# letitiabanana/PnP-OVSS

Measured on AMD Instinct MI355X. Metric: images/sec (336^2, drop_iter=4, blur+CRF), higher is better.
Workload: dtype bf16x3

## Files before the change

### pnp-ovss_amd/csrc/gemm_x3.hip

```cpp
#include <mutex>
#include <type_traits>

#include "common.h"
#include "gemm.h"
#include "gemm_wide.h"

namespace pnp {

typedef __attribute__((ext_vector_type(4))) uint32_t frag16;

__device__ __forceinline__ void x3_half(f32x4& c0, f32x4& c1, const frag16& ah, const frag16& al, const frag16& bh0, const frag16& bh1,
                                        const frag16& bl0, const frag16& bl1) {
    asm volatile(
        "v_mfma_f32_16x16x32_bf16 %0, %6, %2, %0\n\t"
        "v_mfma_f32_16x16x32_bf16 %1, %7, %2, %1\n\t"
        "v_mfma_f32_16x16x32_bf16 %0, %4, %3, %0\n\t"
        "v_mfma_f32_16x16x32_bf16 %1, %5, %3, %1\n\t"
        "v_mfma_f32_16x16x32_bf16 %0, %4, %2, %0\n\t"
        "v_mfma_f32_16x16x32_bf16 %1, %5, %2, %1"
        : "+v"(c0), "+v"(c1)
        : "v"(ah), "v"(al), "v"(bh0), "v"(bh1), "v"(bl0), "v"(bl1));
}

typedef __attribute__((ext_vector_type(4))) uint32_t u32x4;
typedef __attribute__((address_space(1))) uint32_t gu32;
constexpr int kSkAux = 16;

template <int EPI, bool SK>
__global__ __launch_bounds__(512) void gemm_nt_x3_kernel(const GemmArgs g) {
    constexpr int BM = 256, BN = 256, SLOT = 65536, ARR = 16384;
    constexpr int JM = 8, IN = 4;
    constexpr int NDMA = 8;
    constexpr int kDrain = (EPI == WIDE_GELU_SPLIT || EPI == WIDE_SPLIT) ? 32 : 24;
    constexpr int SROW = kWideStageRow;
    extern __shared__ __attribute__((aligned(16))) char smem[];

    const int tid = threadIdx.x;
    const int lane = tid & 63, wave = __builtin_amdgcn_readfirstlane(tid >> 6);
    const int r = lane & 15, q = lane >> 4;
    const int wm = wave >> 2, wn = wave & 3;
    const int nbm = (g.M + BM - 1) / BM, nbn = g.N / BN;
    const int ntiles = nbm * nbn;
    const int nk = g.K / 32;
    const char* Ab = reinterpret_cast<const char*>(g.A);
    const char* Bb = reinterpret_cast<const char*>(g.B);
    const char* Alo = reinterpret_cast<const char*>(g.A_lo);
    const char* Blo = reinterpret_cast<const char*>(g.B_lo);

    uint32_t soff[4];
    auto set_tile = [&](int tile, int& m0, int& n0, int lane) {
        int bm, bn;
        tile_coords<4>(tile, nbm, nbn, bm, bn);
        m0 = bm * BM;
        n0 = bn * BN;
        const uint32_t lda_b = (uint32_t)g.lda * 2, ldb_b = (uint32_t)g.ldb * 2;
        const int c = (lane & 3) ^ ((-(lane >> 4)) & 3);
#pragma unroll
        for (int i = 0; i < 2; i++) {
            const int row = (wave * 2 + i) * 16 + (lane >> 2);
            int gr = m0 + row;
            gr = gr < g.M ? gr : g.M - 1;
            soff[i] = (uint32_t)gr * lda_b + c * 16;
            gr = n0 + row;
            gr = gr < g.Nvalid ? gr : g.Nvalid - 1;
            soff[2 + i] = (uint32_t)gr * ldb_b + c * 16;
        }
    };
    auto issue_one = [&](int kt, int i, uint32_t on) {
        const int op = i >> 2, rg = (i >> 1) & 1, lo = i & 1;
        const char* base = op ? (lo ? Blo : Bb) : (lo ? Alo : Ab);
        const int d = (kt & 1) * SLOT + op * (2 * ARR) + lo * ARR + (wave * 2 + rg) * 1024;
        const uint32_t lds = (uint32_t)(uintptr_t)(__attribute__((address_space(3))) char*)(smem + d);
        uint32_t voff;
        uint64_t saved;
        asm volatile(
            "s_mov_b64 %1, exec\n\t"
            "s_cmp_lg_u32 %6, 0\n\t"
            "s_cselect_b64 exec, exec, 0\n\t"
            "v_add_u32 %0, %3, %2\n\t"
            "s_mov_b32 m0, %5\n\t"
            "s_nop 0\n\t"
            "global_load_lds_dwordx4 %0, %4\n\t"
            "s_mov_b64 exec, %1"
            : "=&v"(voff), "=&s"(saved)
            : "v"(soff[op * 2 + rg]), "s"((uint32_t)kt * 64), "s"(base), "s"(lds), "s"(on)
            : "memory", "scc");
    };
    auto stamp_sk = [&](int slot) {
        if (g.stamps && tid == 0) {
            g.stamps[((size_t)gridDim.x + blockIdx.x) * 8 + slot] = __builtin_readcyclecounter();
            g.stamps[((size_t)gridDim.x + blockIdx.x) * 8 + 4 + slot] = wall_clock64();
        }
    };
    auto stamp = [&](int slot) {
        if (g.stamps && tid == 0) {
            g.stamps[(size_t)blockIdx.x * 8 + slot] = __builtin_readcyclecounter();
            g.stamps[(size_t)blockIdx.x * 8 + 4 + slot] = wall_clock64();
        }
    };

    const int fo = r * 64 + ((q ^ ((-(r >> 2)) & 3)) << 4);
    int fa_off[2], fb_off[2];
    fa_off[0] = wm * (128 * 64) + fo;
    fb_off[0] = 2 * ARR + wn * (64 * 64) + fo;
    fa_off[1] = fa_off[0] + SLOT;
    fb_off[1] = fb_off[0] + SLOT;
    asm volatile("" : "+v"(fa_off[1]), "+v"(fb_off[1]));
    float* const stg = reinterpret_cast<float*>(smem + SLOT) + wave * (32 * SROW);

    const int bid = blockIdx.x;
    enum { kWhole = 0, kProduce = 1, kOwn = 2 };
    auto get_work = [&](int wi, int& t, int& k0, int& k1, int& kind) {
        const int grid = gridDim.x;
        const int full = SK ? g.sk_full : ntiles;
        t = bid + wi * grid;
        if (t < full) {
            k0 = 0;
            k1 = nk;
            kind = kWhole;
            return true;
        }
        if constexpr (SK) {
            const int j = wi - g.sk_full / grid;
            const int nk2 = nk >> 1;
            const int T = (ntiles - full) * nk2;
            const int u0 = bid * g.sk_upw;
            const int u1 = u0 + g.sk_upw < T ? u0 + g.sk_upw : T;
            if (u0 >= u1 || j > 1) return false;
            const int ta = u0 / nk2, bnd = (ta + 1) * nk2;
            const bool owns = u1 >= bnd, two = u1 > bnd;
            if (j == 0 && (two || !owns)) {
                t = full + ta + (two ? 1 : 0);
                k0 = two ? 0 : 2 * (u0 - ta * nk2);
                k1 = 2 * (u1 - (two ? bnd : ta * nk2));
                kind = kProduce;
                return true;
            }
            if (owns && (j == 0 || two)) {
                t = full + ta;
                k0 = 2 * (u0 - ta * nk2);
                k1 = nk;
                kind = k0 ? kOwn : kWhole;
                return true;
            }
        }
        return false;
    };
    int wi = 0, tile, k0, k1, kind;
    if (!get_work(0, tile, k0, k1, kind)) return;
    int m0, n0;
    bool drain32 = false;
    stamp(0);
    set_tile(tile, m0, n0, lane);
#pragma unroll
    for (int i = 0; i < NDMA; i++) issue_one(k0, i, 1u);

    for (;;) {
        f32x4 acc[JM][IN];
#pragma unroll
        for (int j = 0; j < JM; j++)
#pragma unroll
            for (int i = 0; i < IN; i++) acc[j][i] = f32x4{0.f, 0.f, 0.f, 0.f};

        frag16 ah[4], al[4], bh[2][IN], bl[2][IN];
        auto rd_a = [&](int slot, int s, int jm) {
            const char* p = smem + fa_off[s] + jm * 1024;
            ah[slot] = *reinterpret_cast<const frag16*>(p);
            al[slot] = *reinterpret_cast<const frag16*>(p + ARR);
        };
        auto rd_b = [&](int set, int s, int in) {
            const char* p = smem + fb_off[s] + in * 1024;
            bh[set][in] = *reinterpret_cast<const frag16*>(p);
            bl[set][in] = *reinterpret_cast<const frag16*>(p + ARR);
        };

        if (drain32) PNP_WAIT_VM(kDrain);
        else PNP_WAIT_VM(0);
        __builtin_amdgcn_s_barrier();
#pragma unroll
        for (int i = 0; i < NDMA; i++) issue_one(k0 + 1, i, 1u);
        rd_a(0, 0, 0);
        rd_a(1, 0, 1);
        rd_a(2, 0, 2);
#pragma unroll
        for (int i = 0; i < IN; i++) rd_b(0, 0, i);

        auto slab = [&](int kt, auto par) {
            constexpr int S = decltype(par)::value;
            const uint32_t head = __builtin_amdgcn_readfirstlane((kt >= k0 + 1 && kt + 1 < k1) ? 1 : 0);
            const uint32_t tail = __builtin_amdgcn_readfirstlane((kt + 2 < k1) ? 1 : 0);
#pragma unroll
            for (int j = 0; j < JM; j++) {
                x3_half(acc[j][0], acc[j][1], ah[j & 3], al[j & 3], bh[S][0], bh[S][1], bl[S][0], bl[S][1]);
                if (j + 3 < JM) {
                    rd_a((j + 3) & 3, S, j + 3);
                    if (j < 2) issue_one(kt + 1, 4 + 2 * j, head);
                } else {
                    if (j == JM - 3) {
                        __builtin_amdgcn_s_waitcnt(0x0070);
                        __builtin_amdgcn_s_barrier();
                    }
                    rd_a((j + 3) & 3, S ^ 1, j + 3 - JM);
                    if (j == JM - 2) rd_b(S ^ 1, S ^ 1, 1);
                    if (j == JM - 1) rd_b(S ^ 1, S ^ 1, 3);
                    if (j == JM - 3) issue_one(kt + 2, 0, tail);
                    if (j == JM - 2) issue_one(kt + 2, 2, tail);
                }
                x3_half(acc[j][2], acc[j][3], ah[j & 3], al[j & 3], bh[S][2], bh[S][3], bl[S][2], bl[S][3]);
                if (j < 2) issue_one(kt + 1, 5 + 2 * j, head);
                if (j == JM - 3) {
                    rd_b(S ^ 1, S ^ 1, 0);
                    issue_one(kt + 2, 1, tail);
                }
                if (j == JM - 2) {
                    rd_b(S ^ 1, S ^ 1, 2);
                    issue_one(kt + 2, 3, tail);
                }
            }
        };
        constexpr std::integral_constant<int, 0> s0{};
        constexpr std::integral_constant<int, 1> s1{};
        for (int kt = k0; kt < k1; kt += 2) {
            slab(kt, s0);
            slab(kt + 1, s1);
        }
        asm volatile("s_nop 15\n\ts_nop 15" ::: "memory");
        if (wi == 0) stamp(2);

        __syncthreads();
        int ntile, nk0, nk1, nkind;
        const bool have_next = get_work(wi + 1, ntile, nk0, nk1, nkind);
        auto request_next = [&]() {
            if (have_next) {
                set_tile(ntile, m0, n0, lane);
#pragma unroll
                for (int i = 0; i < NDMA; i++) issue_one(nk0, i, 1u);
            }
        };
        if constexpr (SK) {
            if (kind == kProduce) {
                stamp_sk(0);
                request_next();
                const __amdgpu_buffer_rsrc_t rs = __builtin_amdgcn_make_buffer_rsrc(g.sk_part + (size_t)bid * (BM * BN), 0, BM * BN * 4, 0x00020000);
                {
                    int voff = tid * 16;
#pragma unroll
                    for (int j = 0; j < JM; j++)
#pragma unroll
                        for (int i = 0; i < IN; i++) {
                            __builtin_amdgcn_raw_buffer_store_b128(__builtin_bit_cast(u32x4, acc[j][i]), rs, voff, 0, kSkAux);
                            voff += 8192;
                            asm volatile("" : "+v"(voff));
                        }
                }
                asm volatile("s_waitcnt vmcnt(0)" ::: "memory");
                __syncthreads();
                if (tid == 0) __hip_atomic_store((gu32*)(g.sk_flag + bid), 1u, __ATOMIC_RELAXED, __HIP_MEMORY_SCOPE_AGENT);
                stamp_sk(1);
            }
            if (kind == kOwn) {
                const int np = ((k0 >> 1) + g.sk_upw - 1) / g.sk_upw;
                stamp_sk(2);
                for (int pj = 1; pj <= np; pj++) {
                    const int src = bid - pj;
                    if (wave == 0) {
                        gu32* const fl = (gu32*)(g.sk_flag + src);
                        uint32_t spins = 0;
                        while (__hip_atomic_load(fl, __ATOMIC_RELAXED, __HIP_MEMORY_SCOPE_AGENT) != 1u) {
                            __builtin_amdgcn_s_sleep(8);
                            if (++spins > (1u << 22)) {
                                if (lane == 0) __hip_atomic_store((gu32*)g.sk_tmo, 1u + (uint32_t)bid, __ATOMIC_RELAXED, __HIP_MEMORY_SCOPE_AGENT);
                                break;
                            }
                        }
                        if (lane == 0) __hip_atomic_store(fl, 0u, __ATOMIC_RELAXED, __HIP_MEMORY_SCOPE_AGENT);
                    }
                    __syncthreads();
                    const __amdgpu_buffer_rsrc_t rs = __builtin_amdgcn_make_buffer_rsrc(g.sk_part + (size_t)src * (BM * BN), 0, BM * BN * 4, 0x00020000);
                    int voff = tid * 16;
#pragma unroll
                    for (int grp = 0; grp < 4; grp++) {
                        u32x4 t[8];
#pragma unroll
                        for (int x = 0; x < 8; x++) {
                            t[x] = __builtin_amdgcn_raw_buffer_load_b128(rs, voff, 0, kSkAux);
                            voff += 8192;
                            asm volatile("" : "+v"(voff));
                        }
#pragma unroll
                        for (int x = 0; x < 8; x++) acc[(grp * 8 + x) / IN][(grp * 8 + x) % IN] += __builtin_bit_cast(f32x4, t[x]);
                    }
                }
                stamp_sk(3);
            }
        }
        bool next_drain = false;
        if (!SK || kind != kProduce) {
        int etid = tid;
        asm volatile("" : "+v"(etid));
        const int lane = etid & 63, r = lane & 15, q = lane >> 4;
        const int em0 = m0, en0 = n0;
        const int n = en0 + wn * 64 + (lane & 15) * 4;
        const bool nv = n < g.Nvalid;
        f32x4 bv = {0.f, 0.f, 0.f, 0.f};
        f32x4 rv[8];
        f32x4 bacc[IN];
        if constexpr (EPI == WIDE_GELU_SPLIT || EPI == WIDE_SPLIT) {
#pragma unroll
            for (int i = 0; i < IN; i++) {
                const int nn = en0 + wn * 64 + i * 16 + q * 4;
                bacc[i] = (g.bias && nn < g.Nvalid) ? *reinterpret_cast<const f32x4*>(g.bias + nn) : bv;
            }
        }
        if constexpr (EPI == WIDE_BIAS_F32 || EPI == WIDE_RESID_F32) {
            if (g.bias && nv) bv = *reinterpret_cast<const f32x4*>(g.bias + n);
        }
        if constexpr (EPI == WIDE_RESID_F32) {
            const int mrow0 = em0 + wm * 128 + (lane >> 4);
#pragma unroll
            for (int it = 0; it < 8; it++) {
                const int m = mrow0 + it * 4;
                rv[it] = (m < g.M && nv) ? *reinterpret_cast<const f32x4*>(g.resid + (size_t)m * g.ldr + n) : bv;
            }
        }
        float brow[JM] = {0.f, 0.f, 0.f, 0.f, 0.f, 0.f, 0.f, 0.f};
        if constexpr (EPI == WIDE_TOKCOLS_F32) {
#pragma unroll
            for (int j = 0; j < JM; j++) {
                const int m = em0 + wm * 128 + j * 16 + r;
                if (g.bias && m < g.M) brow[j] = g.bias[m];
            }
        }

        if constexpr (EPI == WIDE_TOKCOLS_F32) {
            const int l32 = lane & 31, hi = lane >> 5;
            const bool pairs = (g.col_div & 1) == 0;
            const int tl0 = pairs ? 2 * l32 : lane;
            const int tok = en0 + wn * 64 + tl0;
            size_t ocol = tok;
            if (g.col_div > 0) {
                const int b = tok / g.col_div;
                const int tl = tok - b * g.col_div;
                ocol = (size_t)b * g.col_pad + tl;
            }
            float* const ocolp = g.out_f32 + ocol;
            const bool tv = tok < g.Nvalid;
#pragma unroll
            for (int qd = 0; qd < 4; qd++) {
                const int mbase = em0 + wm * 128 + qd * 32;
#pragma unroll
                for (int j2 = 0; j2 < 2; j2++)
#pragma unroll
                    for (int i = 0; i < IN; i++) {
                        const float br = brow[qd * 2 + j2];
                        const f32x4 v = acc[qd * 2 + j2][i] + br;
                        *reinterpret_cast<f32x4*>(stg + (j2 * 16 + r) * SROW + i * 16 + q * 4) = v;
                    }
                if (qd == 0) request_next();
                if (pairs) {
                    f32x2 sv[16];
#pragma unroll
                    for (int it = 0; it < 16; it++) sv[it] = *reinterpret_cast<const f32x2*>(stg + (it * 2 + hi) * SROW + tl0);
#pragma unroll
                    for (int it = 0; it < 16; it++) {
                        const int m = mbase + it * 2 + hi;
                        if (tv && m < g.M) *reinterpret_cast<f32x2*>(ocolp + (size_t)m * g.ldo) = sv[it];
                    }
                } else {
#pragma unroll 8
                    for (int row = 0; row < 32; row++) {
                        const float v = stg[row * SROW + lane];
                        if (tv && mbase + row < g.M) ocolp[(size_t)(mbase + row) * g.ldo] = v;
                    }
                }
            }
        } else if constexpr (EPI == WIDE_GELU_SPLIT || EPI == WIDE_SPLIT) {
            constexpr int HROW = 68;
            bf16* const stgh = reinterpret_cast<bf16*>(smem + SLOT) + wave * (64 * HROW);
            const bool full = (em0 + BM <= g.M) && (en0 + BN <= g.Nvalid);
#pragma unroll
            for (int half = 0; half < 2; half++) {
#pragma unroll
                for (int j4 = 0; j4 < 4; j4++)
#pragma unroll
                    for (int i = 0; i < IN; i++)
#pragma unroll
                        for (int e = 0; e < 4; e += 2) {
                            f32x4& a = acc[half * 4 + j4][i];
                            pnp_f32x2 v = {a[e] + bacc[i][e], a[e + 1] + bacc[i][e + 1]};
                            if constexpr (EPI == WIDE_GELU_SPLIT) v = gelu_erf_fast2(v);
                            a[e] = v[0];
                            a[e + 1] = v[1];
                        }
                if (half == 0) request_next();
#pragma unroll
                for (int part = 0; part < 2; part++) {
                    bf16* const obase = reinterpret_cast<bf16*>(part ? g.out_lo : g.out_t) + (size_t)(em0 + wm * 128 + (lane >> 4)) * g.ldo_t + n;
#pragma unroll
                    for (int j4 = 0; j4 < 4; j4++)
#pragma unroll
                        for (int i = 0; i < IN; i++) {
                            const f32x4& a = acc[half * 4 + j4][i];
                            bf16x4 pk;
#pragma unroll
                            for (int e = 0; e < 4; e++) {
                                const float v = a[e];
                                const bf16 h = (bf16)v;
                                pk[e] = part ? (bf16)(v - (float)h) : h;
                            }
                            *reinterpret_cast<bf16x4*>(stgh + (j4 * 16 + r) * HROW + i * 16 + q * 4) = pk;
                        }
                    bf16x4 sv[16];
#pragma unroll
                    for (int it = 0; it < 16; it++)
                        sv[it] = *reinterpret_cast<const bf16x4*>(stgh + (it * 4 + (lane >> 4)) * HROW + (lane & 15) * 4);
#pragma unroll
                    for (int it = 0; it < 16; it++) {
                        const int m = em0 + wm * 128 + half * 64 + it * 4 + (lane >> 4);
                        if (full || (m < g.M && nv)) *reinterpret_cast<bf16x4*>(obase + (size_t)(half * 64 + it * 4) * g.ldo_t) = sv[it];
                    }
                }
            }
        } else {
            constexpr bool kResid = EPI == WIDE_RESID_F32;
            const bool full = (em0 + BM <= g.M) && (en0 + BN <= g.Nvalid);
            const float* const rbase = kResid ? g.resid + (size_t)(em0 + wm * 128 + (lane >> 4)) * g.ldr + n : nullptr;
            float* const obase = g.out_f32 + (size_t)(em0 + wm * 128 + (lane >> 4)) * g.ldo + n;
            f32x4 rw[8];
#pragma unroll
            for (int qd = 0; qd < 4; qd++) {
                f32x4* const rcur = (qd & 1) ? rw : rv;
                f32x4* const rnxt = (qd & 1) ? rv : rw;
#pragma unroll
                for (int j2 = 0; j2 < 2; j2++)
#pragma unroll
                    for (int i = 0; i < IN; i++)
                        *reinterpret_cast<f32x4*>(stg + (j2 * 16 + r) * SROW + i * 16 + q * 4) = acc[qd * 2 + j2][i];
                if (kResid && qd < 3) {
#pragma unroll
                    for (int it = 0; it < 8; it++) {
                        const int m = em0 + wm * 128 + (qd + 1) * 32 + it * 4 + (lane >> 4);
                        rnxt[it] = (full || (m < g.M && nv)) ? *reinterpret_cast<const f32x4*>(rbase + (size_t)((qd + 1) * 32 + it * 4) * g.ldr) : bv;
                    }
                }
                f32x4 sv[8];
#pragma unroll
                for (int it = 0; it < 8; it++)
                    sv[it] = *reinterpret_cast<const f32x4*>(stg + (it * 4 + (lane >> 4)) * SROW + (lane & 15) * 4);
#pragma unroll
                for (int it = 0; it < 8; it++) {
                    f32x4 v = sv[it] + bv;
                    if constexpr (kResid) v += rcur[it];
                    const int m = em0 + wm * 128 + qd * 32 + it * 4 + (lane >> 4);
                    if (full || (m < g.M && nv)) *reinterpret_cast<f32x4*>(obase + (size_t)(qd * 32 + it * 4) * g.ldo) = v;
                }
                if (qd == 0) request_next();
            }
        }
        next_drain = (EPI != WIDE_TOKCOLS_F32) && (em0 + BM <= g.M) && (en0 + BN <= g.Nvalid);
        }
        if (wi == 0) stamp(1);
        if (!have_next) break;
        wi++;
        tile = ntile;
        k0 = nk0;
        k1 = nk1;
        kind = nkind;
        drain32 = next_drain;
    }
    if (g.stamps) {
        asm volatile("s_waitcnt vmcnt(0)" ::: "memory");
        stamp(3);
    }
}

static std::atomic<int> g_streamk_mode{1};
void set_streamk_mode(int m) { g_streamk_mode.store(m, std::memory_order_relaxed); }
int streamk_mode() { return g_streamk_mode.load(std::memory_order_relaxed); }
static std::mutex g_sk_chain_mu;
static hipEvent_t g_sk_chain_last[kMaxDevices];
int streamk_chain_launch(GemmKernel kernel, const GemmArgs& g, int grid, StreamKWs* ws, hipStream_t s) {
    const int d = current_device();
    if (d < 0) return PNP_ERR_HIP;
    std::lock_guard<std::mutex> lk(g_sk_chain_mu);
    hipEvent_t& last = g_sk_chain_last[d];
    ws->launches++;
    if (!last) {
        if (hipEventCreateWithFlags(&last, hipEventDisableTiming) != hipSuccess) return PNP_ERR_HIP;
    } else if (hipStreamWaitEvent(s, last, 0) != hipSuccess) {
        return PNP_ERR_HIP;
    }
    hipLaunchKernelGGL(kernel, dim3(grid), dim3(512), kWideSmem, s, g);
    const bool ok = hipGetLastError() == hipSuccess && hipEventRecord(last, s) == hipSuccess;
    return ok ? PNP_OK : PNP_ERR_HIP;
}

int streamk_ws_create(StreamKWs* ws, int wgs) {
    if (!ws || wgs <= 0) return PNP_ERR_ARG;
    const size_t fbytes = ((size_t)(wgs + 1) * 4 + 15) / 16 * 16;
    if (hipMalloc(&ws->part, (size_t)wgs * 256 * 256 * 4) != hipSuccess) return PNP_ERR_HIP;
    if (hipMalloc(&ws->flag, fbytes) != hipSuccess || hipMemset(ws->flag, 0, fbytes) != hipSuccess) {
        (void)hipFree(ws->part);
        ws->part = nullptr;
        return PNP_ERR_HIP;
    }
    ws->wgs = wgs;
    return PNP_OK;
}

void streamk_ws_destroy(StreamKWs* ws) {
    if (!ws) return;
    if (ws->part) (void)hipFree(ws->part);
    if (ws->flag) (void)hipFree(ws->flag);
    *ws = StreamKWs();
}

int streamk_ws_timeouts(StreamKWs* ws, unsigned* out) {
    if (!ws || !out) return PNP_ERR_ARG;
    *out = 0;
    if (!ws->flag) return PNP_OK;
    return hipMemcpy(out, ws->flag + ws->wgs, 4, hipMemcpyDeviceToHost) == hipSuccess ? PNP_OK : PNP_ERR_HIP;
}

StreamKWs* streamk_ws_default() {
    static StreamKWs ws[kMaxDevices];
    static std::mutex mu;
    const int d = current_device();
    if (d < 0) return nullptr;
    std::lock_guard<std::mutex> lk(mu);
    if (!ws[d].part) {
        const int n = device_cu_count();
        if (!n || streamk_ws_create(&ws[d], n) != PNP_OK) return nullptr;
    }
    return &ws[d];
}

GemmKernel gemm_x3_kernel(int epi, int sk) {
#define X3_CASE(E) case E: return sk ? gemm_nt_x3_kernel<E, true> : gemm_nt_x3_kernel<E, false>
    switch (epi) { X3_CASE(WIDE_RESID_F32); X3_CASE(WIDE_BIAS_F32); X3_CASE(WIDE_TOKCOLS_F32); X3_CASE(WIDE_GELU_SPLIT); X3_CASE(WIDE_SPLIT); }
#undef X3_CASE
    return nullptr;
}

}
```

Baseline: 222.3.

## Permute B rows in split-output GEMM so epilogue stores directly without LDS staging

For the GELU/split epilogues, the B operand rows are loaded in a permuted order so each lane's accumulator columns become contiguous groups of 8. The epilogue then writes the bf16 hi/lo pairs straight to global memory as 16-byte vectors, which removes the per-wave LDS staging round trip and its barrier-free shuffle. The bias indexing is remapped to match the permutation. The cost is row-strided global stores (each lane writes its own row) in place of the fully coalesced row-major pattern, and the stores are only 8-byte aligned.

```diff
diff --git a/pnp-ovss_amd/csrc/gemm_x3.hip b/pnp-ovss_amd/csrc/gemm_x3.hip
--- a/pnp-ovss_amd/csrc/gemm_x3.hip
+++ b/pnp-ovss_amd/csrc/gemm_x3.hip
@@ -31,7 +31,8 @@
     constexpr int BM = 256, BN = 256, SLOT = 65536, ARR = 16384;
     constexpr int JM = 8, IN = 4;
     constexpr int NDMA = 8;
-    constexpr int kDrain = (EPI == WIDE_GELU_SPLIT || EPI == WIDE_SPLIT) ? 32 : 24;
+    constexpr bool kPair = EPI == WIDE_GELU_SPLIT || EPI == WIDE_SPLIT;
+    constexpr int kDrain = kPair ? 32 : 24;
     constexpr int SROW = kWideStageRow;
     extern __shared__ __attribute__((aligned(16))) char smem[];
 
@@ -61,7 +62,8 @@
             int gr = m0 + row;
             gr = gr < g.M ? gr : g.M - 1;
             soff[i] = (uint32_t)gr * lda_b + c * 16;
-            gr = n0 + row;
+            const int prow = kPair ? (row & ~63) + ((row & 32) | ((row & 12) << 1) | ((row & 16) >> 2) | (row & 3)) : row;
+            gr = n0 + prow;
             gr = gr < g.Nvalid ? gr : g.Nvalid - 1;
             soff[2 + i] = (uint32_t)gr * ldb_b + c * 16;
         }
@@ -305,10 +307,10 @@
         f32x4 bv = {0.f, 0.f, 0.f, 0.f};
         f32x4 rv[8];
         f32x4 bacc[IN];
-        if constexpr (EPI == WIDE_GELU_SPLIT || EPI == WIDE_SPLIT) {
+        if constexpr (kPair) {
 #pragma unroll
             for (int i = 0; i < IN; i++) {
-                const int nn = en0 + wn * 64 + i * 16 + q * 4;
+                const int nn = en0 + wn * 64 + (i >> 1) * 32 + q * 8 + (i & 1) * 4;
                 bacc[i] = (g.bias && nn < g.Nvalid) ? *reinterpret_cast<const f32x4*>(g.bias + nn) : bv;
             }
         }
@@ -374,52 +376,48 @@
                     }
                 }
             }
-        } else if constexpr (EPI == WIDE_GELU_SPLIT || EPI == WIDE_SPLIT) {
-            constexpr int HROW = 68;
-            bf16* const stgh = reinterpret_cast<bf16*>(smem + SLOT) + wave * (64 * HROW);
+        } else if constexpr (kPair) {
+            typedef bf16x8 __attribute__((aligned(8))) bf16x8_a8;
             const bool full = (em0 + BM <= g.M) && (en0 + BN <= g.Nvalid);
-#pragma unroll
-            for (int half = 0; half < 2; half++) {
-#pragma unroll
-                for (int j4 = 0; j4 < 4; j4++)
-#pragma unroll
-                    for (int i = 0; i < IN; i++)
-#pragma unroll
-                        for (int e = 0; e < 4; e += 2) {
-                            f32x4& a = acc[half * 4 + j4][i];
-                            pnp_f32x2 v = {a[e] + bacc[i][e], a[e + 1] + bacc[i][e + 1]};
-                            if constexpr (EPI == WIDE_GELU_SPLIT) v = gelu_erf_fast2(v);
-                            a[e] = v[0];
-                            a[e + 1] = v[1];
+            const int nc = en0 + wn * 64 + q * 8;
+            const size_t o0 = (size_t)(em0 + wm * 128 + r) * g.ldo_t + nc;
+#pragma unroll
+            for (int jm = 0; jm < JM; jm++) {
+#pragma unroll
+                for (int i = 0; i < IN; i++)
+#pragma unroll
+                    for (int e = 0; e < 4; e += 2) {
+                        f32x4& a = acc[jm][i];
+                        pnp_f32x2 v = {a[e] + bacc[i][e], a[e + 1] + bacc[i][e + 1]};
+                        if constexpr (EPI == WIDE_GELU_SPLIT) v = gelu_erf_fast2(v);
+                        a[e] = v[0];
+                        a[e + 1] = v[1];
+                    }
+                if (jm == 0) request_next();
+                const bool mv = em0 + wm * 128 + jm * 16 + r < g.M;
+                bf16x8 ph[2], pl[2];
+#pragma unroll
+                for (int h = 0; h < 2; h++)
+#pragma unroll
+                    for (int e = 0; e < 8; e++) {
+                        const float v = acc[jm][2 * h + (e >> 2)][e & 3];
+                        const bf16 hi = (bf16)v;
+                        ph[h][e] = hi;
+                        pl[h][e] = (bf16)(v - (float)hi);
+                    }
+#pragma unroll
+                for (int part = 0; part < 2; part++)
+#pragma unroll
+                    for (int h = 0; h < 2; h++) {
+                        bf16* const d = reinterpret_cast<bf16*>(part ? g.out_lo : g.out_t) + o0 + (size_t)(jm * 16) * g.ldo_t + h * 32;
+                        const bf16x8 pk = part ? pl[h] : ph[h];
+                        if (full) {
+                            *reinterpret_cast<bf16x8_a8*>(d) = pk;
+                        } else if (mv) {
+                            if (nc + h * 32 < g.Nvalid) *reinterpret_cast<bf16x4*>(d) = pk.lo;
+                            if (nc + h * 32 + 4 < g.Nvalid) *reinterpret_cast<bf16x4*>(d + 4) = pk.hi;
                         }
-                if (half == 0) request_next();
-#pragma unroll
-                for (int part = 0; part < 2; part++) {
-                    bf16* const obase = reinterpret_cast<bf16*>(part ? g.out_lo : g.out_t) + (size_t)(em0 + wm * 128 + (lane >> 4)) * g.ldo_t + n;
-#pragma unroll
-                    for (int j4 = 0; j4 < 4; j4++)
-#pragma unroll
-                        for (int i = 0; i < IN; i++) {
-                            const f32x4& a = acc[half * 4 + j4][i];
-                            bf16x4 pk;
-#pragma unroll
-                            for (int e = 0; e < 4; e++) {
-                                const float v = a[e];
-                                const bf16 h = (bf16)v;
-                                pk[e] = part ? (bf16)(v - (float)h) : h;
-                            }
-                            *reinterpret_cast<bf16x4*>(stgh + (j4 * 16 + r) * HROW + i * 16 + q * 4) = pk;
-                        }
-                    bf16x4 sv[16];
-#pragma unroll
-                    for (int it = 0; it < 16; it++)
-                        sv[it] = *reinterpret_cast<const bf16x4*>(stgh + (it * 4 + (lane >> 4)) * HROW + (lane & 15) * 4);
-#pragma unroll
-                    for (int it = 0; it < 16; it++) {
-                        const int m = em0 + wm * 128 + half * 64 + it * 4 + (lane >> 4);
-                        if (full || (m < g.M && nv)) *reinterpret_cast<bf16x4*>(obase + (size_t)(half * 64 + it * 4) * g.ldo_t) = sv[it];
-                    }
-                }
+                    }
             }
         } else {
             constexpr bool kResid = EPI == WIDE_RESID_F32;
```

New measurement: 223.4 (median of 6 runs). Within noise of the previous version (+0.5%).
